# xandercai/JSPSR

Hardware: AMD Instinct MI355X
Metric: Mpixels/sec fwd+bwd, JSPSR x8 on 512^2 DEM tiles (higher is better)
Workload: dtype bf16; 1 GPU; jspsr_r8_img_msk (image+mask guided, 43.87M params), 8 x 512x512 tiles per GPU, train step (fwd + L1/L2/Sobel loss + bwd + grad all-reduce + AdamW); storage policy: bf16 activations / gradients / MFMA operands, fp32 accumulation, BatchNorm statistics, master weights and optimizer, and the generator head (affinity logits + offsets) kept as fp32 planes; tiles_per_gpu=8, tile=512, global_tiles=8, parallelism=dp1, step_mode=eager

## Files before the change

### include/jspsr_hip.h

```cpp
#ifndef JSPSR_HIP_H
#define JSPSR_HIP_H

#include <stddef.h>
#include <stdint.h>

#ifdef __cplusplus
extern "C" {
#endif

#define JSPSR_OK 0
#define JSPSR_EINVAL (-1)
#define JSPSR_EALIGN (-2)

typedef void* jspsr_stream_t;

int jspsr_abi_version(void);
long long jspsr_launch_count(const char* what);
int jspsr_conv_dynamic_queue(int on);
const char* jspsr_last_error(void);

int jspsr_prop_forward_f32(const float* dem, const float* weight, const float* offset,
                           int offset_channels, const float* wk, const float* b0, float scale,
                           float* out, int B, int H, int W, jspsr_stream_t stream);

// ... 105 lines not shown
                       const void* red_x, int red_cstride, const float* red_par, float* red_out, jspsr_stream_t stream);

size_t jspsr_conv2d_wgrad_workspace_bytes(int dtype, int B, int OH, int OW, int Cg, int Cx, int KH, int KW);
int jspsr_conv2d_wgrad_x_affine_ok(int dtype, int B, int OH, int OW, int Cg, int Cx, int KH, int KW, int stride, int pad);
int jspsr_conv2d_wgrad(int dtype, const void* G, int Cg, int g_cstride, int g_coff, const void* X, int Cx,
                       int x_cstride, int x_coff, float* dW, int R, int C, int B, int OH, int OW,
                       int IH, int IW, int KH, int KW, int stride, int pad, int accumulate,
                       const float* x_affine, int x_relu, void* workspace, jspsr_stream_t stream);
int jspsr_conv2d_wgrad_scaled(int dtype, const void* G, int Cg, int g_cstride, int g_coff, const void* X, int Cx,
                              int x_cstride, int x_coff, float* dW, int R, int C, int B, int OH, int OW,
                              int IH, int IW, int KH, int KW, int stride, int pad, int accumulate,
                              const float* x_scale, int x_scale_bstride, void* workspace, jspsr_stream_t stream);

size_t jspsr_reduce_workspace_bytes(int dtype, int C, int nseg);

size_t jspsr_bn_mask_bytes(int dtype, long long npix, int C);
int jspsr_bn_forward(int dtype, const void* x, int x_cs, int x_coff, const void* res, int r_cs, int r_coff,
                     void* y, int y_cs, int y_coff, const float* gamma, const float* beta,
                     float* running_mean, float* running_var, float momentum, float eps, int training,
                     int relu, float res_scale, float* save_mean, float* save_invstd, long long npix, int C,
                     const float* ext_partial, int ext_rows, const float* res_affine, float* affine_out,
                     void* mask_out, void* workspace, jspsr_stream_t stream);

int jspsr_bn_fold(const float* gamma, const float* beta, const float* running_mean, const float* running_var,
                  float eps, float res_scale, int C, float* scale, float* shift, jspsr_stream_t stream);

int jspsr_bn_reduce_params(const float* gamma, const float* beta, const float* save_mean, const float* save_invstd, int C,
                           float* par, jspsr_stream_t stream);
int jspsr_bn_backward(int dtype, const void* dy, int dy_cs, int dy_coff, const void* y, int y_cs, int y_coff,
                      const void* x, int x_cs, int x_coff, const float* gamma, const float* beta, const float* save_mean,
                      const float* save_invstd, int training, int relu, float res_scale, void* dx, void* dres,
                      float* dgamma, float* dbeta, int accumulate, long long npix, int C, void* workspace,
                      const float* ext_partial, int ext_rows, const void* mask, jspsr_stream_t stream);

int jspsr_act_backward(int dtype, const void* dy, int dy_cs, int dy_coff, const void* y, int y_cs, int relu, void* dz,
                       int dz_cs, float* dbias, long long npix, int C, void* workspace, jspsr_stream_t stream);

int jspsr_gate_pool(int dtype, const void* x, int B, long long npix, int C, float* avg, float* mx, int* amax,
                    void* workspace, jspsr_stream_t stream);
int jspsr_gate_scale(int dtype, const void* x, const float* s, void* y, int B, long long npix, int C,
                     jspsr_stream_t stream);
int jspsr_gate_backward_reduce(int dtype, const void* dy, const void* x, float* ds, int B, long long npix, int C,
                               void* workspace, jspsr_stream_t stream);
int jspsr_gate_backward_apply(int dtype, const void* dy, const float* s, const float* davg, const float* dmax,
                              const int* amax, void* dx, int B, long long npix, int C, jspsr_stream_t stream);

size_t jspsr_loss_workspace_bytes(int B, int H, int W);
int jspsr_loss_forward(const float* pred, const float* gt, float w1, float w2, float wg, float* losses,
                       void* workspace, int B, int H, int W, jspsr_stream_t stream);
int jspsr_loss_backward(const float* pred, const float* gt, const float* grad_total, float w1, float w2,
                        float wg, float* grad_pred, const void* workspace, int B, int H, int W,
                        jspsr_stream_t stream);

size_t jspsr_loss_menu_workspace_bytes(int terms, int planes, int H, int W);
int jspsr_loss_menu_forward(const float* pred, const float* gt, int terms, int planes, int H, int W, int n_keys,
                            const int* key_slot, const double* key_weight, const float* base_losses, float* out,
                            void* workspace, jspsr_stream_t stream);
int jspsr_loss_menu_backward(const float* pred, const float* gt, int terms, int planes, int H, int W,
                             const double* slot_weight, const float* grad_total, float* grad_pred,
                             const void* workspace, jspsr_stream_t stream);
size_t jspsr_loss_valid_workspace_bytes(int B, int H, int W);
int jspsr_loss_valid_forward(const float* pred, const float* gt, const unsigned char* valid, float w1, float w2, float wg,
                             float* losses, void* workspace, int B, int H, int W, jspsr_stream_t stream);
int jspsr_loss_valid_backward(const float* pred, const float* gt, const unsigned char* valid, const float* grad_total,
                              float w1, float w2, float wg, float* grad_pred, const void* workspace, int B, int H, int W,
                              jspsr_stream_t stream);
// ... 124 lines not shown
```

### jspsr_amd/_lib.py

```python
from __future__ import annotations

import ctypes
import os
import subprocess
import threading

_HERE = os.path.dirname(os.path.abspath(__file__))
SO_PATH = os.environ.get("JSPSR_LAB_LIB") or os.path.join(_HERE, "lib", "libjspsr_hip.so")
CSRC = os.path.join(_HERE, "csrc")
ABI_VERSION = 25

_lock = threading.Lock()
_lib = None

c_p = ctypes.c_void_p
c_i = ctypes.c_int
c_f = ctypes.c_float
c_ll = ctypes.c_longlong

SIGNATURES = {
    "jspsr_abi_version": (c_i, []),
    "jspsr_launch_count": (c_ll, [ctypes.c_char_p]),
    "jspsr_conv_dynamic_queue": (c_i, [c_i]),
    "jspsr_last_error": (ctypes.c_char_p, []),
# ... 7 lines not shown
    "jspsr_prop_head_forward": (c_i, [c_i, c_p, c_p, c_p, c_p, c_f, c_p, c_i, c_i, c_i, c_p]),
    "jspsr_prop_head_backward_workspace_bytes": (ctypes.c_size_t, [c_i, c_i, c_i]),
    "jspsr_prop_head_backward": (c_i, [c_i] + [c_p] * 8 + [c_i, c_i, c_i, c_p]),
    "jspsr_prop_logits_forward_f32": (c_i, [c_p, c_p, c_p, c_p, c_f, c_p, c_i, c_i, c_i, c_p]),
    "jspsr_prop_logits_backward_f32": (c_i, [c_p] * 8 + [c_i, c_i, c_i, c_p]),
    "jspsr_head_ok": (c_i, [c_i] * 5),
    "jspsr_head_forward": (c_i, [c_i, c_p, c_i, c_i, c_i, c_p, c_p, c_p, c_i, c_i, c_i, c_p]),
    "jspsr_head_backward_workspace_bytes": (ctypes.c_size_t, [c_i, c_i, c_i]),
    "jspsr_head_backward": (c_i, [c_i, c_p, c_p, c_i, c_p, c_i, c_i, c_p, c_p, c_p, c_i, c_i, c_i, c_p]),
    "jspsr_conv_head1_forward": (c_i, [c_i, c_p, c_i, c_i, c_i, c_p, c_p, c_p, c_i, c_i, c_i, c_p]),
    "jspsr_conv_head1_workspace_bytes": (ctypes.c_size_t, [c_i, c_i, c_i, c_i]),
    "jspsr_conv_head1_backward": (c_i, [c_i, c_p, c_p, c_i, c_i, c_i, c_p, c_p, c_i, c_i, c_p, c_p, c_p, c_i, c_i, c_i, c_p]),
    "jspsr_pack_weight": (c_i, [c_i, c_p, c_p] + [c_i] * 6 + [c_p]),
    "jspsr_pack_chunk": (c_i, []),
    "jspsr_pack_weights_multi": (c_i, [c_p, c_i, c_ll, c_p]),
    "jspsr_conv2d_stats_rows": (c_i, [c_i, c_i, c_i]),
    "jspsr_conv2d_in_affine_ok": (c_i, [c_i] * 5),
    "jspsr_conv2d_forward": (c_i, [c_i] + [c_p] * 4 + [c_i] * 14 + [c_p, c_p, c_p, c_i, c_p, c_i, c_p]),
    "jspsr_conv2d_forward_scaled": (c_i, [c_i] + [c_p] * 4 + [c_i] * 14 + [c_p, c_p, c_p, c_i, c_p, c_i, c_p]),
    "jspsr_bn_fold": (c_i, [c_p, c_p, c_p, c_p, c_f, c_f, c_i, c_p, c_p, c_p]),
    "jspsr_conv2d_dgrad_reduce_ok": (c_i, [c_i] * 10),
    "jspsr_conv2d_dgrad": (c_i, [c_i] + [c_p] * 4 + [c_i] * 16 + [c_p, c_i, c_p, c_p, c_i, c_p, c_p, c_p]),
    "jspsr_conv2d_wgrad_workspace_bytes": (ctypes.c_size_t, [c_i] * 8),
    "jspsr_conv2d_wgrad_x_affine_ok": (c_i, [c_i] * 10),
    "jspsr_conv2d_wgrad": (c_i, [c_i, c_p, c_i, c_i, c_i, c_p, c_i, c_i, c_i, c_p] + [c_i] * 12 + [c_p, c_i, c_p, c_p]),
    "jspsr_conv2d_wgrad_scaled": (c_i, [c_i, c_p, c_i, c_i, c_i, c_p, c_i, c_i, c_i, c_p] + [c_i] * 12 + [c_p, c_i, c_p, c_p]),
    "jspsr_reduce_workspace_bytes": (ctypes.c_size_t, [c_i, c_i, c_i]),
    "jspsr_bn_forward": (c_i, [c_i, c_p, c_i, c_i, c_p, c_i, c_i, c_p, c_i, c_i, c_p, c_p, c_p, c_p, c_f, c_f, c_i,
                               c_i, c_f, c_p, c_p, c_ll, c_i, c_p, c_i, c_p, c_p, c_p, c_p, c_p]),
    "jspsr_bn_mask_bytes": (ctypes.c_size_t, [c_i, c_ll, c_i]),
    "jspsr_bn_reduce_params": (c_i, [c_p, c_p, c_p, c_p, c_i, c_p, c_p]),
    "jspsr_bn_backward": (c_i, [c_i, c_p, c_i, c_i, c_p, c_i, c_i, c_p, c_i, c_i, c_p, c_p, c_p, c_p, c_i, c_i, c_f,
                                c_p, c_p, c_p, c_p, c_i, c_ll, c_i, c_p, c_p, c_i, c_p, c_p]),
    "jspsr_act_backward": (c_i, [c_i, c_p, c_i, c_i, c_p, c_i, c_i, c_p, c_i, c_p, c_ll, c_i, c_p, c_p]),
    "jspsr_gate_pool": (c_i, [c_i, c_p, c_i, c_ll, c_i, c_p, c_p, c_p, c_p, c_p]),
    "jspsr_gate_scale": (c_i, [c_i, c_p, c_p, c_p, c_i, c_ll, c_i, c_p]),
    "jspsr_gate_backward_reduce": (c_i, [c_i, c_p, c_p, c_p, c_i, c_ll, c_i, c_p, c_p]),
    "jspsr_gate_backward_apply": (c_i, [c_i, c_p, c_p, c_p, c_p, c_p, c_p, c_i, c_ll, c_i, c_p]),
    "jspsr_loss_workspace_bytes": (ctypes.c_size_t, [c_i, c_i, c_i]),
    "jspsr_loss_forward": (c_i, [c_p, c_p, c_f, c_f, c_f, c_p, c_p, c_i, c_i, c_i, c_p]),
    "jspsr_loss_backward": (c_i, [c_p, c_p, c_p, c_f, c_f, c_f, c_p, c_p, c_i, c_i, c_i, c_p]),
    "jspsr_loss_menu_workspace_bytes": (ctypes.c_size_t, [c_i, c_i, c_i, c_i]),
    "jspsr_loss_menu_forward": (c_i, [c_p, c_p, c_i, c_i, c_i, c_i, c_i, c_p, c_p, c_p, c_p, c_p, c_p]),
    "jspsr_loss_menu_backward": (c_i, [c_p, c_p, c_i, c_i, c_i, c_i, c_p, c_p, c_p, c_p, c_p]),
    "jspsr_loss_valid_workspace_bytes": (ctypes.c_size_t, [c_i, c_i, c_i]),
    "jspsr_loss_valid_forward": (c_i, [c_p, c_p, c_p, c_f, c_f, c_f, c_p, c_p, c_i, c_i, c_i, c_p]),
    "jspsr_loss_valid_backward": (c_i, [c_p, c_p, c_p, c_p, c_f, c_f, c_f, c_p, c_p, c_i, c_i, c_i, c_p]),
    "jspsr_loss_menu_valid_workspace_bytes": (ctypes.c_size_t, [c_i, c_i, c_i, c_i]),
    "jspsr_loss_menu_valid_forward": (c_i, [c_p, c_p, c_p, c_i, c_i, c_i, c_i, c_i, c_p, c_p, c_p, c_p, c_p, c_p]),
    "jspsr_loss_menu_valid_backward": (c_i, [c_p, c_p, c_p, c_i, c_i, c_i, c_i, c_p, c_p, c_p, c_p, c_p]),
    "jspsr_ssim_workspace_bytes": (ctypes.c_size_t, [c_i, c_i, c_i, c_i]),
    "jspsr_ssim_forward": (c_i, [c_p, c_p, c_i, c_i, c_i, c_i, c_p, c_p, c_p, c_p]),
    "jspsr_metrics_workspace_bytes": (ctypes.c_size_t, [c_i, c_i]),
    "jspsr_metrics_forward": (c_i, [c_p, c_p, c_i, c_i, c_f, c_f, c_f, c_i, c_p, c_p, c_p]),
    "jspsr_scores_batch_workspace_bytes": (ctypes.c_size_t, [c_i, c_i, c_i]),
    "jspsr_scores_batch_forward": (c_i, [c_p, c_p, c_i, c_i, c_i, c_f, c_f, c_f, c_i, c_p, c_p, c_p]),
    "jspsr_scores_batch_valid_workspace_bytes": (ctypes.c_size_t, [c_i, c_i, c_i]),
    "jspsr_scores_batch_valid_forward": (c_i, [c_p, c_p, c_p, c_i, c_i, c_i, c_f, c_f, c_f, c_i, c_p, c_p, c_p, c_p]),
    "jspsr_scenes_assemble_f32": (c_i, [c_p] * 5 + [c_ll] + [c_i] * 6 + [ctypes.c_double, ctypes.c_double, c_p]),
    "jspsr_summary_workspace_bytes": (ctypes.c_size_t, [c_i, c_i, c_ll, c_ll]),
    "jspsr_summary_forward": (c_i, [c_p, c_p, c_i, c_p, c_ll, c_p, c_i, c_p, c_i, c_ll, c_ll, ctypes.c_double, c_p, c_p, c_p]),
    "jspsr_summary_valid_workspace_bytes": (ctypes.c_size_t, [c_i, c_i, c_ll, c_ll]),
    "jspsr_summary_valid_forward": (c_i, [c_p, c_p, c_i, c_p, c_ll, c_p, c_ll, c_p, c_i, c_p, c_i, c_ll, c_ll, ctypes.c_double,
                                          c_p, c_p, c_p, c_p]),
    "jspsr_summary_ranks": (c_i, [c_ll, c_p]),
    "jspsr_errdist_bins": (c_i, [ctypes.c_double, ctypes.c_double, c_p, c_p]),
# ... 86 lines not shown
```

### jspsr_amd/csrc/elementwise.hip

```cpp
#include "common.h"

#include <atomic>
#include <cstdlib>

namespace {

using namespace jspsr;

constexpr int TX = 64, TY = 4;

template <typename T> struct V;
template <> struct V<float> { static constexpr int N = 4; };
template <> struct V<__bf16> { static constexpr int N = 8; };

template <typename T, int N>
struct Pack { T v[N]; };

template <typename T>
__device__ __forceinline__ uint4 load_raw(const T* p) { return *reinterpret_cast<const uint4*>(p); }
template <typename T>
__device__ __forceinline__ void unpack(const uint4& raw, float (&f)[V<T>::N]) {
  if constexpr (sizeof(T) == 4) {
    f[0] = __uint_as_float(raw.x); f[1] = __uint_as_float(raw.y); f[2] = __uint_as_float(raw.z); f[3] = __uint_as_float(raw.w);
  } else {
// ... 109 lines not shown
    long long p = p0 + ty * g.pl + lm.sub;
    for (; p + (PIX_FLY - 1) * step < p1; p += PIX_FLY * step) {
      uint4 raw[PIX_FLY][NTEN];
#pragma unroll
      for (int u = 0; u < PIX_FLY; ++u) load(base + p + u * step, c, raw[u]);
#pragma unroll
      for (int u = 0; u < PIX_FLY; ++u) use(base + p + u * step, c, raw[u], acc);
    }
    for (; p < p1; p += step) {
      uint4 raw[NTEN];
      load(base + p, c, raw);
      use(base + p, c, raw, acc);
    }
  }
#pragma unroll
  for (int k = 0; k < K; ++k)
#pragma unroll
    for (int i = 0; i < N; ++i) red[ty][k][tx * N + i] = acc[k][i];
  __syncthreads();
  if (ty == 0 && lm.sub == 0 && c < g.C) {
    float* dst = partial + ((size_t)blockIdx.x * K) * g.C + c;
#pragma unroll
    for (int k = 0; k < K; ++k)
#pragma unroll
      for (int i = 0; i < N; ++i) {
        float s = 0.f;
        for (int j = 0; j < g.pl; ++j)
#pragma unroll
          for (int y = 0; y < TY; ++y) s += red[y][k][(tx + j * g.lpp) * N + i];
        dst[(size_t)k * g.C + i] = s;
      }
  }
}
template <typename T, int NTEN, typename L, typename F>
__device__ __forceinline__ void for_pixels_mlp(const RedGeom& g, L&& load, F&& use) {
  constexpr int N = V<T>::N;
  const LaneMap lm = lane_map<N>(g);
  const int c = lm.c;
  if (c >= g.C) return;
  const int seg = blockIdx.x / g.chunks, chunk = blockIdx.x % g.chunks;
  const long long p0 = chunk * g.chunk_pix;
  const long long p1 = (p0 + g.chunk_pix < g.npix) ? p0 + g.chunk_pix : g.npix;
  const long long step = TY * g.pl, base = (long long)seg * g.npix;
  long long p = p0 + threadIdx.y * g.pl + lm.sub;
  for (; p + (PIX_FLY - 1) * step < p1; p += PIX_FLY * step) {
    uint4 raw[PIX_FLY][NTEN];
#pragma unroll
    for (int u = 0; u < PIX_FLY; ++u) load(base + p + u * step, c, raw[u]);
#pragma unroll
    for (int u = 0; u < PIX_FLY; ++u) use(p + u * step, base + p + u * step, c, raw[u]);
  }
  for (; p < p1; p += step) {
    uint4 raw[NTEN];
    load(base + p, c, raw);
    use(p, base + p, c, raw);
  }
}

template <int N>
__device__ __forceinline__ void load_param(const float* __restrict__ p, float (&f)[N]) {
#pragma unroll
  for (int i = 0; i < N; i += 4) {
    const float4 v = *reinterpret_cast<const float4*>(p + i);
    f[i] = v.x; f[i + 1] = v.y; f[i + 2] = v.z; f[i + 3] = v.w;
  }
}

__device__ __forceinline__ double wave_sum_rows(const float* __restrict__ partial, int rows, size_t pitch, size_t off) {
  const int lane = threadIdx.x & 63;
  double s = 0.0;
  for (int r = lane; r < rows; r += 64) s += (double)partial[(size_t)r * pitch + off];
#pragma unroll
  for (int d = 32; d > 0; d >>= 1) s += __shfl_xor(s, d, 64);
  return s;
}

__device__ __forceinline__ void wave_sum_rows2(const float* __restrict__ partial, int rows, size_t pitch, size_t off0, size_t off1,
                                               double& s0, double& s1) {
  const int lane = threadIdx.x & 63;
  double a = 0.0, b = 0.0;
  int r = lane;
  for (; r + 192 < rows; r += 256) {
    const float x0 = partial[(size_t)r * pitch + off0], x1 = partial[(size_t)(r + 64) * pitch + off0];
// ... 218 lines not shown
  constexpr int N = V<T>::N, NTEN = (RELU == 1 || RELU == 3) ? 3 : 2;
  const int C = g.C, groups = C / N;
  float mu[N], is[N], k0[N], ka[N], kb[N], ga[N], be[N];
  const int c0 = lane_map<N>(g).c;
  if (c0 < C) {
    load_param<N>(mean + c0, mu); load_param<N>(invstd + c0, is);
    load_param<N>(coef + c0, k0); load_param<N>(coef + C + c0, ka); load_param<N>(coef + 2 * C + c0, kb);
    if (RELU == 2) { load_param<N>(gamma + c0, ga); load_param<N>(beta + c0, be); }
  }
  for_pixels_mlp<T, NTEN>(
      g,
      [&](long long pix, int c, uint4 (&raw)[NTEN]) {
        raw[0] = load_raw<T>(dy + (size_t)pix * dy_cs + dy_coff + c);
        raw[1] = load_raw<T>(x + (size_t)pix * x_cs + x_coff + c);
        if constexpr (RELU == 1) raw[2] = load_raw<T>(y + (size_t)pix * y_cs + y_coff + c);
        if constexpr (RELU == 3) raw[2].x = mask[(size_t)pix * groups + c / N];
      },
      [&](long long, long long pix, int c, const uint4 (&raw)[NTEN]) {
        float d[N], xv[N], yv[N], o[N];
        unpack<T>(raw[0], d);
        unpack<T>(raw[1], xv);
        if constexpr (RELU == 1) unpack<T>(raw[2], yv);
#pragma unroll
        for (int k = 0; k < N; ++k) {
          const float xhat = (xv[k] - mu[k]) * is[k];
          const bool off = RELU == 1 ? !(yv[k] > 0.f)
                                     : (RELU == 2 ? !(ga[k] * xhat + be[k] > 0.f) : (RELU == 3 ? !((raw[2].x >> k) & 1u) : false));
          const float dz = off ? 0.f : d[k];
          d[k] = dz;
          o[k] = k0[k] * (dz - ka[k] - xhat * kb[k]);
        }
        store_vec<T>(dx + (size_t)pix * C + c, o);
        if (dres) store_vec<T>(dres + (size_t)pix * C + c, d);
      });
}

template <typename T, bool RELU>
__global__ __launch_bounds__(TX * TY) void act_bwd_kernel(const T* __restrict__ dy, int dy_cs, int dy_coff,
                                                         const T* __restrict__ y, int y_cs, int relu,
                                                         T* __restrict__ dz, int dz_cs, RedGeom g,
                                                         float* __restrict__ partial) {
  constexpr int N = V<T>::N;
  constexpr int NTEN = RELU ? 2 : 1;
  (void)relu;
  reduce_pixels_mlp<T, 1, NTEN>(
      g, partial,
      [&](long long pix, int c, uint4 (&raw)[NTEN]) {
        raw[0] = load_raw<T>(dy + (size_t)pix * dy_cs + dy_coff + c);
        if constexpr (RELU) raw[1] = load_raw<T>(y + (size_t)pix * y_cs + c);
      },
      [&](long long pix, int c, const uint4 (&raw)[NTEN], float (&acc)[1][N]) {
        float d[N], yv[N];
        unpack<T>(raw[0], d);
        if constexpr (RELU) unpack<T>(raw[1], yv);
#pragma unroll
        for (int i = 0; i < N; ++i) {
          if (RELU && !(yv[i] > 0.f)) d[i] = 0.f;
          acc[0][i] += d[i];
        }
        if (dz) store_vec<T>(dz + (size_t)pix * dz_cs + c, d);
      });
}

__global__ void sum_rows_kernel(const float* __restrict__ partial, int rows, int K, int k, int C, float* __restrict__ out) {
  const int c = blockIdx.x * (blockDim.x >> 6) + (threadIdx.x >> 6);
  if (c >= C) return;
// ... 307 lines not shown
    if (ext_rows <= 0) return fail(JSPSR_EINVAL, "bn_backward: ext_rows must be positive");
    if (ext_rows > 1024) {
      rows = g.chunks < 1024 ? (g.chunks > 0 ? g.chunks : 1) : 1024;
      hipLaunchKernelGGL(fold_rows_kernel, dim3(rows, (2 * C + 255) / 256), dim3(256), 0, s, ext_partial, ext_rows, 2 * C, rows, partial);
      if (int e = check_launch("bn_fold_rows")) return e;
    } else {
      partial = const_cast<float*>(ext_partial);
      rows = ext_rows;
    }
  } else {
    if (mode == 0) { BN_BWD_REDUCE(0, false); }
    else if (mode == 2) { BN_BWD_REDUCE(2, false); }
    else if (mode == 1) { if (premask) { BN_BWD_REDUCE(1, true); } else { BN_BWD_REDUCE(1, false); } }
    else { if (premask) { BN_BWD_REDUCE(3, true); } else { BN_BWD_REDUCE(3, false); } }
    if (int e = check_launch("bn_bwd_reduce")) return e;
  }
#undef BN_BWD_REDUCE
  hipLaunchKernelGGL(bn_bwd_finalize_kernel, dim3((C + 3) / 4), dim3(256), 0, s, partial, rows, C, npix, gamma,
                     save_invstd, training, res_scale, accumulate, dgamma, dbeta, coef);
  if (int e = check_launch("bn_bwd_finalize")) return e;
#define BN_BWD_APPLY(R, DY, CS, OFF, DRES) DISPATCH(dtype, hipLaunchKernelGGL((bn_bwd_apply_kernel<T, R>), red_grid(g, vec), dim3(TX, TY), 0, s, \
                                     static_cast<const T*>(DY), CS, OFF, static_cast<const T*>(y), y_cs, y_coff,            \
                                     static_cast<const T*>(x), x_cs, x_coff, save_mean, save_invstd, gamma, beta, coef, mk, \
                                     static_cast<T*>(dx), static_cast<T*>(DRES), g))
  if (premask) { BN_BWD_APPLY(0, dres, C, 0, nullptr); }
  else if (mode == 0) { BN_BWD_APPLY(0, dy, dy_cs, dy_coff, dres); }
  else if (mode == 1) { BN_BWD_APPLY(1, dy, dy_cs, dy_coff, dres); }
  else if (mode == 2) { BN_BWD_APPLY(2, dy, dy_cs, dy_coff, dres); }
  else { BN_BWD_APPLY(3, dy, dy_cs, dy_coff, dres); }
#undef BN_BWD_APPLY
  return check_launch("bn_bwd_apply");
}

extern "C" int jspsr_bn_fold(const float* gamma, const float* beta, const float* running_mean, const float* running_var,
                             float eps, float res_scale, int C, float* scale, float* shift, jspsr_stream_t stream) {
  if (!gamma || !beta || !running_mean || !running_var || !scale || !shift || C <= 0)
    return fail(JSPSR_EINVAL, "bn_fold: bad arguments");
  hipLaunchKernelGGL(bn_fold_kernel, dim3((C + 255) / 256), dim3(256), 0, static_cast<hipStream_t>(stream), gamma, beta,
                     running_mean, running_var, eps, res_scale, C, scale, shift);
  return check_launch("bn_fold");
}

extern "C" int jspsr_act_backward(int dtype, const void* dy, int dy_cs, int dy_coff, const void* y, int y_cs, int relu,
                                  void* dz, int dz_cs, float* dbias, long long npix, int C, void* workspace,
                                  jspsr_stream_t stream) {
  if (int e = check_c(dtype, C, "act_backward")) return e;
  if (!dy || (relu && !y) || !workspace || npix <= 0) return fail(JSPSR_EINVAL, "act_backward: null pointer or empty tensor");
  const int vec = dtype == JSPSR_F32 ? 4 : 8;
  if (dy_cs % vec || dy_coff % vec || (dz && dz_cs % vec) || (relu && (y_cs % vec || y_cs < C)))
    return fail(JSPSR_EINVAL, "act_backward: bad pitch");
  hipStream_t s = static_cast<hipStream_t>(stream);
  float* partial = static_cast<float*>(workspace);
  const RedGeom g = make_red(npix, 1, C, vec);
#define ACT_BWD(R) DISPATCH(dtype, hipLaunchKernelGGL((act_bwd_kernel<T, R>), red_grid(g, vec), dim3(TX, TY), 0, s, static_cast<const T*>(dy), \
                                     dy_cs, dy_coff, static_cast<const T*>(y), y_cs, relu, static_cast<T*>(dz), dz_cs, g, partial))
  if (relu) { ACT_BWD(true); } else { ACT_BWD(false); }
#undef ACT_BWD
  if (int e = check_launch("act_backward")) return e;
  if (dbias) {
    hipLaunchKernelGGL(sum_rows_kernel, dim3((C + 3) / 4), dim3(256), 0, s, partial, g.chunks, 1, 0, C, dbias);
    return check_launch("act_backward_bias");
  }
  return JSPSR_OK;
}

extern "C" int jspsr_gate_pool(int dtype, const void* x, int B, long long npix, int C, float* avg, float* mx, int* amax,
// ... 395 lines not shown
```

### jspsr_amd/kernels.py

```python
from __future__ import annotations

import torch

from . import _lib

F32, BF16 = 0, 1


def _dt(t: torch.Tensor) -> int:
    if t.dtype == torch.float32:
        return F32
    if t.dtype == torch.bfloat16:
        return BF16
    raise TypeError(f"unsupported dtype {t.dtype}")


def epc(dtype: torch.dtype) -> int:
    return 4 if dtype == torch.float32 else 8


def _stream() -> int:
    return torch.cuda.current_stream().cuda_stream


# ... 153 lines not shown
                 x_affine=None, x_relu=False, x_scale=None):
    _chk_s(G, "conv2d_wgrad")
    _chk_s(X, "conv2d_wgrad")
    B, OH, OW, Cg_ = G.shape
    _, IH, IW, Cx_ = X.shape
    Cgs, Cxs = pitch(G), pitch(X)
    cg = Cg_ if cg is None else cg
    cx = Cx_ if cx is None else cx
    if out is None:
        out = torch.empty((R, C, KH, KW), dtype=torch.float32, device=G.device)
    lib = _lib.load()
    dt = _dt(G)
    nbytes = lib.jspsr_conv2d_wgrad_workspace_bytes(dt, B, OH, OW, cg, cx, KH, KW)
    ws = torch.empty(max(nbytes, 16), dtype=torch.uint8, device=G.device)
    head = (dt, G.data_ptr(), cg, Cgs, g_coff, X.data_ptr(), cx, Cxs, x_coff, out.data_ptr(), R, C, B, OH, OW, IH, IW, KH, KW,
            stride, pad, int(accumulate))
    if x_scale is not None:
        if x_affine is not None:
            raise ValueError("conv2d_wgrad: x_scale and x_affine exclude each other")
        _chk_scale(x_scale, B, cx, "conv2d_wgrad x_scale")
        _lib.check(lib.jspsr_conv2d_wgrad_scaled(*head, x_scale.data_ptr(), x_scale.shape[1], ws.data_ptr(), _stream()),
                   "jspsr_conv2d_wgrad_scaled")
    else:
        _lib.check(lib.jspsr_conv2d_wgrad(*head, x_affine.data_ptr() if x_affine is not None else None, int(x_relu),
                                          ws.data_ptr(), _stream()), "jspsr_conv2d_wgrad")
    return out



_ws_cache = {}


def _workspace(dtype_code: int, C: int, nseg: int, device) -> torch.Tensor:
    lib = _lib.load()
    n = lib.jspsr_reduce_workspace_bytes(dtype_code, C, nseg)
    key = (device, _stream())
    buf = _ws_cache.get(key)
    if buf is None or buf.numel() < n:
        buf = torch.empty(max(n, 1 << 20), dtype=torch.uint8, device=device)
        _ws_cache[key] = buf
    return buf


def bn_forward(x, gamma, beta, running_mean, running_var, momentum, eps, training, relu=False, res=None,
               res_scale=1.0, out=None, out_coff=0, partial=None, res_affine=None, stats_only=False, want_mask=False):
    _chk_s(x, "bn_forward")
    B, H, W, C = x.shape
    affine = torch.empty((2, C), dtype=torch.float32, device=x.device) if stats_only else None
    if out is None and not stats_only:
        out = torch.empty((B, H, W, C), dtype=x.dtype, device=x.device)
    mean = torch.empty(C, dtype=torch.float32, device=x.device)
    invstd = torch.empty(C, dtype=torch.float32, device=x.device)
    dt = _dt(x)
    ws = _workspace(dt, C, 1, x.device)
    lib = _lib.load()
    mask = torch.empty(lib.jspsr_bn_mask_bytes(dt, B * H * W, C), dtype=torch.uint8, device=x.device) if want_mask else None
    _lib.check(lib.jspsr_bn_forward(dt, x.data_ptr(), pitch(x), 0, res.data_ptr() if res is not None else None,
                                    pitch(res) if res is not None else 0, 0, out.data_ptr() if out is not None else None,
                                    pitch(out) if out is not None else 0, out_coff,
                                    gamma.data_ptr(), beta.data_ptr(),
                                    running_mean.data_ptr() if running_mean is not None else None,
                                    running_var.data_ptr() if running_var is not None else None,
                                    float(momentum), float(eps), int(training), int(relu), float(res_scale),
                                    mean.data_ptr(), invstd.data_ptr(), B * H * W, C,
                                    partial.data_ptr() if partial is not None else None,
                                    partial.shape[0] if partial is not None else 0,
                                    res_affine.data_ptr() if res_affine is not None else None,
                                    affine.data_ptr() if affine is not None else None,
# ... 18 lines not shown
                grads_into=None, ext_partial=None, mask=None):
    _chk_s(dy, "bn_backward")
    B, H, W, C = x.shape
    dx = torch.empty((B, H, W, C), dtype=x.dtype, device=x.device)
    dres = torch.empty((B, H, W, C), dtype=x.dtype, device=x.device) if want_dres else None
    if grads_into is not None:
        dgamma, dbeta = grads_into
        for t in (dgamma, dbeta):
            if t.dtype != torch.float32 or not t.is_contiguous() or t.numel() != C or not t.is_cuda:
                raise ValueError("bn_backward: grads_into buffers must be contiguous fp32 of C elements on the GPU")
    else:
        dgamma = torch.empty(C, dtype=torch.float32, device=x.device)
        dbeta = torch.empty(C, dtype=torch.float32, device=x.device)
    dt = _dt(x)
    ws = _workspace(dt, C, 1, x.device)
    lib = _lib.load()
    if mask is not None and (mask.dtype != torch.uint8 or not mask.is_contiguous() or
                             mask.numel() != lib.jspsr_bn_mask_bytes(dt, B * H * W, C)):
        raise ValueError("bn_backward: mask is not the bit mask bn_forward(want_mask=True) made for this shape")
    _lib.check(lib.jspsr_bn_backward(dt, dy.data_ptr(), pitch(dy), 0, y.data_ptr() if y is not None else None,
                                     pitch(y) if y is not None else 0, 0, x.data_ptr(), pitch(x), 0, gamma.data_ptr(),
                                     beta.data_ptr() if beta is not None else None,
                                     mean.data_ptr(), invstd.data_ptr(), int(training), int(relu), float(res_scale),
                                     dx.data_ptr(), dres.data_ptr() if dres is not None else None, dgamma.data_ptr(),
                                     dbeta.data_ptr(), int(grads_into is not None), B * H * W, C, ws.data_ptr(),
                                     ext_partial.data_ptr() if ext_partial is not None else None,
                                     ext_partial.shape[0] if ext_partial is not None else 0,
                                     mask.data_ptr() if mask is not None else None, _stream()), "jspsr_bn_backward")
    if grads_into is not None:
        return dx, dres, None, None
    return dx, dres, dgamma, dbeta


def act_backward(dy, y, relu, want_dz=True, want_dbias=True, dz_channels=None):
    _chk_s(dy, "act_backward")
    B, H, W, C = dy.shape
    dz = None
    if want_dz:
        cz = C if dz_channels is None else dz_channels
        dz = torch.empty((B, H, W, cz), dtype=dy.dtype, device=dy.device) if cz == C else \
            torch.zeros((B, H, W, cz), dtype=dy.dtype, device=dy.device)
    dbias = torch.empty(C, dtype=torch.float32, device=dy.device) if want_dbias else None
    dt = _dt(dy)
    ws = _workspace(dt, C, 1, dy.device)
    lib = _lib.load()
    if y is not None:
        y = nhwc(y)
    _lib.check(lib.jspsr_act_backward(dt, dy.data_ptr(), pitch(dy), 0, y.data_ptr() if y is not None else None,
                                      pitch(y) if y is not None else 0, int(relu),
                                      dz.data_ptr() if dz is not None else None, dz.shape[3] if dz is not None else 0,
                                      dbias.data_ptr() if dbias is not None else None, B * H * W, C, ws.data_ptr(),
                                      _stream()), "jspsr_act_backward")
    return dz, dbias


def gate_pool(x):
    _chk(x, "gate_pool")
    B, H, W, C = x.shape
    avg = torch.empty((B, C), dtype=torch.float32, device=x.device)
    mx = torch.empty_like(avg)
    amax = torch.empty((B, C), dtype=torch.int32, device=x.device)
    dt = _dt(x)
    ws = _workspace(dt, C, B, x.device)
    lib = _lib.load()
    _lib.check(lib.jspsr_gate_pool(dt, x.data_ptr(), B, H * W, C, avg.data_ptr(), mx.data_ptr(), amax.data_ptr(),
                                   ws.data_ptr(), _stream()), "jspsr_gate_pool")
# ... 71 lines not shown
```

### jspsr_amd/ops.py

```python
from __future__ import annotations

import collections
import os
import weakref

import torch

from . import _lib
from . import kernels as K


def _stream() -> int:
    return torch.cuda.current_stream().cuda_stream


def _need_gpu(*ts):
    for t in ts:
        if not t.is_cuda:
            raise RuntimeError("jspsr_amd ops run on the GPU only (got a CPU tensor); there is no CPU fallback")
        if t.dtype != torch.float32:
            raise TypeError(f"expected float32, got {t.dtype}")


def prop_forward_raw(dem, weight, offset, w, b, scale, out):
# ... 465 lines not shown
    _, table, grand = _pack_table
    _lib.check(_lib.load().jspsr_pack_weights_multi(table.data_ptr(), len(entries), grand, _stream()), "jspsr_pack_weights_multi")
    for p, mode, c_pad, dtype, packed in entries:
        p.__dict__["_jspsr_packs"][(mode, c_pad, dtype, p.data_ptr())] = (packed, (p._version, _weights_epoch))
    return len(entries)


def pad_channels(x: torch.Tensor, mult: int) -> torch.Tensor:
    c = x.shape[-1]
    p = (-c) % mult
    return x if p == 0 else torch.nn.functional.pad(x, (0, p))


def _wgrad_into(param, G, X, R, C, KH, KW, stride, pad, **kw):
    gbuf = param.grad if param is not None and getattr(param, "_jspsr_direct_grad", False) else None
    if (gbuf is not None and gbuf.dtype == torch.float32 and gbuf.is_contiguous() and gbuf.is_cuda
            and tuple(gbuf.shape) == (R, C, KH, KW)):
        K.conv2d_wgrad(G, X, R, C, KH, KW, stride, pad, out=gbuf, accumulate=True, **kw)
        ready = getattr(param, "_jspsr_grad_ready", None)
        if ready is not None:
            ready(param)
        return None
    return K.conv2d_wgrad(G, X, R, C, KH, KW, stride, pad, **kw)


_aux_streams = {}
_marks = {}
RUN_AHEAD = int(os.environ.get("JSPSR_RUN_AHEAD", "16"))
wgrad_async = os.environ.get("JSPSR_WGRAD_ASYNC", "1") != "0"
wgrad_after_dgrad = os.environ.get("JSPSR_WGRAD_AFTER_DGRAD", "0") != "0"
wgrad_one_stream = os.environ.get("JSPSR_WGRAD_ONE_STREAM", "0") != "0"
bn_reduce_fused = os.environ.get("JSPSR_BN_REDUCE_FUSE", "1") != "0"
bn_relu_mask = os.environ.get("JSPSR_BN_RELU_MASK", "1") != "0"


def aux_streams():
    return list(_aux_streams.values())


def _wgrad_async(param, G, X, R, C, KH, KW, stride, pad, **kw):
    if not wgrad_async:
        return _wgrad_into(param, G, X, R, C, KH, KW, stride, pad, **kw)
    cur = torch.cuda.current_stream()
    key = 0 if wgrad_one_stream else cur.cuda_stream
    aux = _aux_streams.get(key)
    if aux is None:
        aux = _aux_streams[key] = torch.cuda.Stream(device=G.device)
    aux.wait_stream(cur)
    with torch.cuda.stream(aux):
        dW = _wgrad_into(param, G, X, R, C, KH, KW, stride, pad, **kw)
    for t_ in kw.values():
        if isinstance(t_, torch.Tensor):
            t_.record_stream(aux)
    G.record_stream(aux)
    X.record_stream(aux)
    if not torch.cuda.is_current_stream_capturing():
        marks = _marks.setdefault(cur.cuda_stream, collections.deque())
        marks.append(cur.record_event())
        if len(marks) > RUN_AHEAD:
            marks.popleft().synchronize()
    if dW is not None:
        cur.wait_stream(aux)
        dW.record_stream(cur)
    return dW


# ... 249 lines not shown
                r = zd
            else:
                zd, r, md, idd = conv_bn(x, wdd, 1, stride, 0, gdd, bdd, rmd, rvd, momd, epsd, trd, False, par=wd)
                r_aff = None
        else:
            r_aff = None
            if stride != 1 or O != I:
                raise ValueError("res_unit: identity shortcut needs stride 1 and equal channel counts")
            wdd = gdd = bdd = zd = md = idd = None
            trd = False
            r = x
        out_v = dest[0].slice(dest[1], O, z1.shape[:3]) if dest is not None else None
        masked = bool(act) and bn_relu_mask
        z2, out, m2, i2, *mk2 = conv_bn(z1 if fuse1 else y1, w2d, 3, 1, 1, g2d, b2d, rm2, rv2, mom2, eps2, tr2, bool(act), r, float(scale),
                                        out_v, par=w2, res_affine=r_aff, in_affine=aff1, want_mask=masked)
        ctx.cfg = (stride, float(scale), bool(act), has_d, tr1, tr2, trd)
        ctx.wparams = tuple(p if isinstance(p, torch.nn.Parameter) else None for p in (w1, w2, wd))
        ctx.bparams = tuple(p if isinstance(p, torch.nn.Parameter) else None for p in (g1, b1, g2, b2, gd, bd))
        ctx.save_for_backward(x, w1d, g1d, b1d, z1, m1, i1, y1, w2d, g2d, b2d, z2, m2, i2, out if act and not masked else None,
                              wdd, gdd, bdd, zd, md, idd, aff1, mk2[0] if masked else None)
        return out

    @staticmethod
    def backward(ctx, dout):
        stride, scale, act, has_d, tr1, tr2, trd = ctx.cfg
        (x, w1, g1, b1, z1, m1, i1, y1, w2, g2, b2, z2, m2, i2, out, wd, gd, bd, zd, md, idd, aff1, mask2) = ctx.saved_tensors
        cdt = x.dtype
        B, H, W, Cin = x.shape
        O = w1.shape[0]
        dout = K.nhwc(dout)
        need_x = ctx.needs_input_grad[0]
        pg1, pb1, pg2, pb2, pgd, pbd = ctx.bparams
        sink2, sink1 = _bn_sink(pg2, pb2), _bn_sink(pg1, pb1)
        dz2, dres, dg2, db2 = K.bn_backward(dout, out, z2, g2, m2, i2, tr2, 1 if act else 0, scale,
                                            want_dres=(need_x or has_d), beta=b2, grads_into=sink2, mask=mask2)
        if sink2 is not None:
            _bn_ready(pg2, pb2)
        if dres is None:
            dres = dout
        p1, p2, pd = ctx.wparams

        def wgrad2():
            if aff1 is not None:
                return _wgrad_async(p2, dz2, z1, O, O, 3, 3, 1, 1, x_affine=aff1, x_relu=True)
            return _wgrad_async(p2, dz2, y1, O, O, 3, 3, 1, 1)

        if not wgrad_after_dgrad:
            dW2 = wgrad2()
        Bz, Hz, Wz, _ = z1.shape
        part1 = None
        if bn_reduce_fused and tr1 and K.dgrad_reduce_ok(cdt, Bz, Hz, Wz, O, O, 3, 3, 1, 1) and z1.is_contiguous():
            par1 = K.bn_reduce_params(g1, b1, m1, i1)
            dy1, part1 = K.conv2d_dgrad(dz2, _packed(p2, w2, 1, O, cdt), z1.shape[1:3], 1, 1, red=(z1, par1))
        else:
            dy1 = K.conv2d_dgrad(dz2, _packed(p2, w2, 1, O, cdt), z1.shape[1:3], 1, 1)
        if wgrad_after_dgrad:
            dW2 = wgrad2()
        del dz2
        dz1, _, dg1, db1 = K.bn_backward(dy1, None, z1, g1, m1, i1, tr1, 2, 1.0, beta=b1, grads_into=sink1, ext_partial=part1)
        if sink1 is not None:
            _bn_ready(pg1, pb1)
        del dy1
        dW1 = None if wgrad_after_dgrad else _wgrad_async(p1, dz1, x, O, Cin, 3, 3, stride, 1)
        dWd = dgd = dbd = None
        side = dres
        deposit = None
        if isinstance(ctx.grad_extra, tuple):
            holder, off, n = ctx.grad_extra
            if holder.deferred is not None and has_d and need_x:
                cur = torch.cuda.current_stream()
                cur.wait_event(holder.deferred_event)
                deposit = holder.deferred.narrow(3, off, n)
                if tuple(deposit.shape) != tuple(x.shape):
                    raise RuntimeError(f"res_unit: parked gradient slice {tuple(deposit.shape)} does not match the input {tuple(x.shape)}")
                if deposit.dtype != x.dtype or not (deposit.is_contiguous() or K.is_slice(deposit)):
                    holder.pending_deposits -= 1
                    deposit = None
                else:
                    deposit.record_stream(cur)
            elif holder.deferred is not None:
                holder.pending_deposits -= 1
        extra = ctx.grad_extra.take_deferred() if (ctx.grad_extra is not None and not isinstance(ctx.grad_extra, tuple)) else deposit
        if extra is not None:
            extra = K.nhwc(extra)
            if tuple(extra.shape) != tuple(x.shape):
                raise RuntimeError(f"res_unit: deferred gradient {tuple(extra.shape)} does not match the input {tuple(x.shape)}")
            if not (has_d and need_x):
                side, extra = side + extra, None
        if has_d:
            sinkd = _bn_sink(pgd, pbd)
            dzd, _, dgd, dbd = K.bn_backward(dres, None, zd, gd, md, idd, trd, 0, 1.0, beta=bd, grads_into=sinkd)
            if sinkd is not None:
                _bn_ready(pgd, pbd)
            dWd = _wgrad_async(pd, dzd, x, O, Cin, 1, 1, stride, 0)
            side = K.conv2d_dgrad(dzd, _packed(pd, wd, 1, O, cdt), (H, W), stride, 0, addend=extra) if need_x else None
        dx = None
        if need_x and deposit is not None:
            K.conv2d_dgrad(dz1, _packed(p1, w1, 1, O, cdt), (H, W), stride, 1, addend=K.nhwc(side), out=deposit)
            ctx.grad_extra[0].deposit_events.append(torch.cuda.current_stream().record_event())
        elif need_x:
            dx = K.conv2d_dgrad(dz1, _packed(p1, w1, 1, O, cdt), (H, W), stride, 1, addend=K.nhwc(side))
        if wgrad_after_dgrad:
            dW1 = _wgrad_async(p1, dz1, x, O, Cin, 3, 3, stride, 1)
        return (dx, dW1, dg1, db1, dW2, dg2, db2, dWd, dgd, dbd, None, None, None, None, None, None)


def conv_bn_infer(x, weight, gamma, beta, bn, stride, pad, relu=False, res=None, res_scale=1.0, dest=None):
    x = K.nhwc(x)
    rm, rv, _, eps, training = bn
    if training or rm is None:
        raise RuntimeError("conv_bn_infer: BatchNorm must be in eval mode with running statistics")
    sc, sh = K.bn_fold(gamma.detach(), beta.detach(), rm, rv, eps, res_scale if res is not None else 1.0)
    O, I, KH, KW = weight.shape
    B, H, W, Cp = x.shape
    out = None
    if dest is not None:
        out = dest[0].slice(dest[1], O, (B, (H + 2 * pad - KH) // stride + 1, (W + 2 * pad - KW) // stride + 1))
    return K.conv2d_forward(x, _packed(weight, weight.detach().contiguous(), 0, Cp, x.dtype), sh, stride, pad, relu, out=out,
                            scale=sc, addend=K.nhwc(res) if res is not None else None)


def conv_transpose_bn_infer(x, weight, gamma, beta, bn, relu=True, dest=None):
    x = K.nhwc(x)
    rm, rv, _, eps, training = bn
# ... 127 lines not shown
```

Before: 36.64 Mpixel/s.

## Fuse residual-unit output BN and shortcut BN backward into one paired kernel set

In residual units with a downsample shortcut, the backward passes of the second BN and the shortcut BN now run through a single reduce/finalize/apply sequence. That sequence reads dy, the ReLU mask and both pre-BN inputs once. This avoids materialising dres and running a second full BN backward pass over the same gradient. It adds a wider kernel that carries more live registers per thread and more per-channel parameters. It also changes how dgd/dbd and the side gradient are threaded through the Python backward.

```diff
diff --git a/include/jspsr_hip.h b/include/jspsr_hip.h
--- a/include/jspsr_hip.h
+++ b/include/jspsr_hip.h
@@ -161,6 +161,14 @@
                       const float* save_invstd, int training, int relu, float res_scale, void* dx, void* dres,
                       float* dgamma, float* dbeta, int accumulate, long long npix, int C, void* workspace,
                       const float* ext_partial, int ext_rows, const void* mask, jspsr_stream_t stream);
+
+size_t jspsr_bn_backward_pair_workspace_bytes(int dtype, int C);
+int jspsr_bn_backward_pair(int dtype, const void* dy, int dy_cs, int dy_coff, const void* mask, const void* x2, int x2_cs,
+                           int x2_coff, const float* gamma2, const float* save_mean2, const float* save_invstd2,
+                           int training2, float res_scale, const void* xd, int xd_cs, int xd_coff, const float* gammad,
+                           const float* save_meand, const float* save_invstdd, int trainingd, void* dx2, void* dxd,
+                           float* dgamma2, float* dbeta2, int accumulate2, float* dgammad, float* dbetad, int accumulated,
+                           long long npix, int C, void* workspace, jspsr_stream_t stream);
 
 int jspsr_act_backward(int dtype, const void* dy, int dy_cs, int dy_coff, const void* y, int y_cs, int relu, void* dz,
                        int dz_cs, float* dbias, long long npix, int C, void* workspace, jspsr_stream_t stream);
diff --git a/jspsr_amd/_lib.py b/jspsr_amd/_lib.py
--- a/jspsr_amd/_lib.py
+++ b/jspsr_amd/_lib.py
@@ -63,6 +63,9 @@
     "jspsr_bn_reduce_params": (c_i, [c_p, c_p, c_p, c_p, c_i, c_p, c_p]),
     "jspsr_bn_backward": (c_i, [c_i, c_p, c_i, c_i, c_p, c_i, c_i, c_p, c_i, c_i, c_p, c_p, c_p, c_p, c_i, c_i, c_f,
                                 c_p, c_p, c_p, c_p, c_i, c_ll, c_i, c_p, c_p, c_i, c_p, c_p]),
+    "jspsr_bn_backward_pair_workspace_bytes": (ctypes.c_size_t, [c_i, c_i]),
+    "jspsr_bn_backward_pair": (c_i, [c_i, c_p, c_i, c_i, c_p, c_p, c_i, c_i, c_p, c_p, c_p, c_i, c_f, c_p, c_i, c_i, c_p, c_p, c_p, c_i,
+                                     c_p, c_p, c_p, c_p, c_i, c_p, c_p, c_i, c_ll, c_i, c_p, c_p]),
     "jspsr_act_backward": (c_i, [c_i, c_p, c_i, c_i, c_p, c_i, c_i, c_p, c_i, c_p, c_ll, c_i, c_p, c_p]),
     "jspsr_gate_pool": (c_i, [c_i, c_p, c_i, c_ll, c_i, c_p, c_p, c_p, c_p, c_p]),
     "jspsr_gate_scale": (c_i, [c_i, c_p, c_p, c_p, c_i, c_ll, c_i, c_p]),
diff --git a/jspsr_amd/csrc/elementwise.hip b/jspsr_amd/csrc/elementwise.hip
--- a/jspsr_amd/csrc/elementwise.hip
+++ b/jspsr_amd/csrc/elementwise.hip
@@ -165,7 +165,7 @@
       }
   }
 }
-template <typename T, int NTEN, typename L, typename F>
+template <typename T, int NTEN, int FLY = PIX_FLY, typename L, typename F>
 __device__ __forceinline__ void for_pixels_mlp(const RedGeom& g, L&& load, F&& use) {
   constexpr int N = V<T>::N;
   const LaneMap lm = lane_map<N>(g);
@@ -176,12 +176,12 @@
   const long long p1 = (p0 + g.chunk_pix < g.npix) ? p0 + g.chunk_pix : g.npix;
   const long long step = TY * g.pl, base = (long long)seg * g.npix;
   long long p = p0 + threadIdx.y * g.pl + lm.sub;
-  for (; p + (PIX_FLY - 1) * step < p1; p += PIX_FLY * step) {
-    uint4 raw[PIX_FLY][NTEN];
-#pragma unroll
-    for (int u = 0; u < PIX_FLY; ++u) load(base + p + u * step, c, raw[u]);
-#pragma unroll
-    for (int u = 0; u < PIX_FLY; ++u) use(p + u * step, base + p + u * step, c, raw[u]);
+  for (; p + (FLY - 1) * step < p1; p += FLY * step) {
+    uint4 raw[FLY][NTEN];
+#pragma unroll
+    for (int u = 0; u < FLY; ++u) load(base + p + u * step, c, raw[u]);
+#pragma unroll
+    for (int u = 0; u < FLY; ++u) use(p + u * step, base + p + u * step, c, raw[u]);
   }
   for (; p < p1; p += step) {
     uint4 raw[NTEN];
@@ -466,6 +466,123 @@
         }
         store_vec<T>(dx + (size_t)pix * C + c, o);
         if (dres) store_vec<T>(dres + (size_t)pix * C + c, d);
+      });
+}
+
+template <typename T>
+__global__ __launch_bounds__(TX * TY) void bn_bwd_reduce_pair_kernel(const T* __restrict__ dy, int dy_cs, int dy_coff,
+                                                                    const unsigned char* __restrict__ mask,
+                                                                    const T* __restrict__ x2, int x2_cs, int x2_coff,
+                                                                    const float* __restrict__ mean2, const float* __restrict__ invstd2,
+                                                                    const T* __restrict__ xd, int xd_cs, int xd_coff,
+                                                                    const float* __restrict__ meand, const float* __restrict__ invstdd,
+                                                                    RedGeom g, float* __restrict__ partial) {
+  constexpr int N = V<T>::N;
+  const int groups = g.C / N;
+  float mu2[N], is2[N], mud[N], isd[N];
+  const int c0 = lane_map<N>(g).c;
+  if (c0 < g.C) {
+    load_param<N>(mean2 + c0, mu2); load_param<N>(invstd2 + c0, is2);
+    load_param<N>(meand + c0, mud); load_param<N>(invstdd + c0, isd);
+  }
+  reduce_pixels_mlp<T, 3, 4>(
+      g, partial,
+      [&](long long pix, int c, uint4 (&raw)[4]) {
+        raw[0] = load_raw<T>(dy + (size_t)pix * dy_cs + dy_coff + c);
+        raw[1] = load_raw<T>(x2 + (size_t)pix * x2_cs + x2_coff + c);
+        raw[2] = load_raw<T>(xd + (size_t)pix * xd_cs + xd_coff + c);
+        raw[3].x = mask[(size_t)pix * groups + c / N];
+      },
+      [&](long long, int, const uint4 (&raw)[4], float (&acc)[3][N]) {
+        float d[N], xv[N], xw[N];
+        const unsigned m = raw[3].x;
+        unpack<T>(raw[0], d);
+        unpack<T>(raw[1], xv);
+        unpack<T>(raw[2], xw);
+#pragma unroll
+        for (int i = 0; i < N; ++i) {
+          const float xhat = (xv[i] - mu2[i]) * is2[i];
+          const float xhatd = (xw[i] - mud[i]) * isd[i];
+          const float dz = !((m >> i) & 1u) ? 0.f : d[i];
+          acc[0][i] += dz;
+          acc[1][i] += dz * xhat;
+          acc[2][i] += dz * xhatd;
+        }
+      });
+}
+
+__global__ void bn_bwd_finalize_pair_kernel(const float* __restrict__ partial, int rows, int C, long long count,
+                                            const float* __restrict__ gamma2, const float* __restrict__ invstd2, int training2,
+                                            float res_scale, int accumulate2, float* __restrict__ dgamma2, float* __restrict__ dbeta2,
+                                            const float* __restrict__ gammad, const float* __restrict__ invstdd, int trainingd,
+                                            int accumulated, float* __restrict__ dgammad, float* __restrict__ dbetad,
+                                            float* __restrict__ coef) {
+  const int c = blockIdx.x * (blockDim.x >> 6) + (threadIdx.x >> 6);
+  if (c >= C) return;
+  double s, sx;
+  wave_sum_rows2(partial, rows, (size_t)3 * C, c, (size_t)C + c, s, sx);
+  const double sd = wave_sum_rows(partial, rows, (size_t)3 * C, (size_t)2 * C + c);
+  if ((threadIdx.x & 63) != 0) return;
+  auto layer = [&](double sxl, const float* gamma, const float* invstd, int training, float rs, int accumulate,
+                   float* dgamma, float* dbeta, float* co) {
+    dbeta[c] = (accumulate ? dbeta[c] : 0.f) + (float)(s * rs);
+    dgamma[c] = (accumulate ? dgamma[c] : 0.f) + (float)(sxl * rs);
+    const float k = gamma[c] * invstd[c] * rs;
+    co[c] = k;
+    co[C + c] = training ? (float)(s / (double)count) : 0.f;
+    co[2 * C + c] = training ? (float)(sxl / (double)count) : 0.f;
+  };
+  layer(sx, gamma2, invstd2, training2, res_scale, accumulate2, dgamma2, dbeta2, coef);
+  layer(sd, gammad, invstdd, trainingd, 1.0f, accumulated, dgammad, dbetad, coef + 3 * C);
+}
+
+#ifndef K4_PAIR_APPLY_FLY
+#define K4_PAIR_APPLY_FLY 1
+#endif
+constexpr int PAIR_APPLY_FLY = K4_PAIR_APPLY_FLY;
+template <typename T>
+__global__ __launch_bounds__(TX * TY) void bn_bwd_apply_pair_kernel(const T* __restrict__ dy, int dy_cs, int dy_coff,
+                                                                   const unsigned char* __restrict__ mask,
+                                                                   const T* __restrict__ x2, int x2_cs, int x2_coff,
+                                                                   const float* __restrict__ mean2, const float* __restrict__ invstd2,
+                                                                   const T* __restrict__ xd, int xd_cs, int xd_coff,
+                                                                   const float* __restrict__ meand, const float* __restrict__ invstdd,
+                                                                   const float* __restrict__ coef, T* __restrict__ dx2,
+                                                                   T* __restrict__ dxd, RedGeom g) {
+  constexpr int N = V<T>::N;
+  const int C = g.C, groups = C / N;
+  float mu2[N], is2[N], k2[N], a2[N], b2[N], mud[N], isd[N], kd[N], ad[N], bd[N];
+  const int c0 = lane_map<N>(g).c;
+  if (c0 < C) {
+    load_param<N>(mean2 + c0, mu2); load_param<N>(invstd2 + c0, is2);
+    load_param<N>(coef + c0, k2); load_param<N>(coef + C + c0, a2); load_param<N>(coef + 2 * C + c0, b2);
+    load_param<N>(meand + c0, mud); load_param<N>(invstdd + c0, isd);
+    load_param<N>(coef + 3 * C + c0, kd); load_param<N>(coef + 4 * C + c0, ad); load_param<N>(coef + 5 * C + c0, bd);
+  }
+  for_pixels_mlp<T, 4, PAIR_APPLY_FLY>(
+      g,
+      [&](long long pix, int c, uint4 (&raw)[4]) {
+        raw[0] = load_raw<T>(dy + (size_t)pix * dy_cs + dy_coff + c);
+        raw[1] = load_raw<T>(x2 + (size_t)pix * x2_cs + x2_coff + c);
+        raw[2] = load_raw<T>(xd + (size_t)pix * xd_cs + xd_coff + c);
+        raw[3].x = mask[(size_t)pix * groups + c / N];
+      },
+      [&](long long, long long pix, int c, const uint4 (&raw)[4]) {
+        float d[N], xv[N], xw[N], o[N], od[N];
+        const unsigned m = raw[3].x;
+        unpack<T>(raw[0], d);
+        unpack<T>(raw[1], xv);
+        unpack<T>(raw[2], xw);
+#pragma unroll
+        for (int k = 0; k < N; ++k) {
+          const float xhat = (xv[k] - mu2[k]) * is2[k];
+          const float xhatd = (xw[k] - mud[k]) * isd[k];
+          const float dz = !((m >> k) & 1u) ? 0.f : d[k];
+          o[k] = k2[k] * (dz - a2[k] - xhat * b2[k]);
+          od[k] = kd[k] * (dz - ad[k] - xhatd * bd[k]);
+        }
+        store_vec<T>(dx2 + (size_t)pix * C + c, o);
+        store_vec<T>(dxd + (size_t)pix * C + c, od);
       });
 }
 
@@ -839,6 +956,50 @@
   return check_launch("bn_bwd_apply");
 }
 
+extern "C" size_t jspsr_bn_backward_pair_workspace_bytes(int dtype, int C) {
+  const size_t base = jspsr_reduce_workspace_bytes(dtype, C, 1);
+  return base ? base + (size_t)2 * C * sizeof(float) : 0;
+}
+
+extern "C" int jspsr_bn_backward_pair(int dtype, const void* dy, int dy_cs, int dy_coff, const void* mask, const void* x2, int x2_cs,
+                                      int x2_coff, const float* gamma2, const float* save_mean2, const float* save_invstd2,
+                                      int training2, float res_scale, const void* xd, int xd_cs, int xd_coff, const float* gammad,
+                                      const float* save_meand, const float* save_invstdd, int trainingd, void* dx2, void* dxd,
+                                      float* dgamma2, float* dbeta2, int accumulate2, float* dgammad, float* dbetad, int accumulated,
+                                      long long npix, int C, void* workspace, jspsr_stream_t stream) {
+  if (int e = check_c(dtype, C, "bn_backward_pair")) return e;
+  if (!dy || !mask || !x2 || !gamma2 || !save_mean2 || !save_invstd2 || !xd || !gammad || !save_meand || !save_invstdd || !dx2 ||
+      !dxd || !dgamma2 || !dbeta2 || !dgammad || !dbetad || !workspace || npix <= 0)
+    return fail(JSPSR_EINVAL, "bn_backward_pair: null pointer or empty tensor");
+  const int vec = dtype == JSPSR_F32 ? 4 : 8;
+  if (dy_cs % vec || dy_coff % vec || x2_cs % vec || x2_coff % vec || xd_cs % vec || xd_coff % vec)
+    return fail(JSPSR_EINVAL, "bn_backward_pair: channel pitches/offsets must be multiples of %d", vec);
+  if (dy_coff < 0 || x2_coff < 0 || xd_coff < 0 || dy_cs < dy_coff + C || x2_cs < x2_coff + C || xd_cs < xd_coff + C)
+    return fail(JSPSR_EINVAL, "bn_backward_pair: a channel slice of %d channels does not fit its pitch", C);
+  if (dx2 == dxd || dgamma2 == dgammad || dbeta2 == dbetad)
+    return fail(JSPSR_EINVAL, "bn_backward_pair: the two layers' outputs must be distinct");
+  for (const void* p : {dy, x2, xd, (const void*)dx2, (const void*)dxd, (const void*)workspace})
+    if (reinterpret_cast<uintptr_t>(p) % 16) return fail(JSPSR_EALIGN, "bn_backward_pair: tensors and workspace must be 16-byte aligned");
+  hipStream_t s = static_cast<hipStream_t>(stream);
+  float* coef = static_cast<float*>(workspace);
+  float* partial = coef + 6 * C;
+  const RedGeom g = make_red(npix, 1, C, vec);
+  const unsigned char* mk = static_cast<const unsigned char*>(mask);
+  DISPATCH(dtype, hipLaunchKernelGGL(bn_bwd_reduce_pair_kernel<T>, red_grid(g, vec), dim3(TX, TY), 0, s, static_cast<const T*>(dy), dy_cs,
+                                     dy_coff, mk, static_cast<const T*>(x2), x2_cs, x2_coff, save_mean2, save_invstd2,
+                                     static_cast<const T*>(xd), xd_cs, xd_coff, save_meand, save_invstdd, g, partial));
+  if (int e = check_launch("bn_bwd_reduce_pair")) return e;
+  hipLaunchKernelGGL(bn_bwd_finalize_pair_kernel, dim3((C + 3) / 4), dim3(256), 0, s, partial, g.chunks, C, npix, gamma2, save_invstd2,
+                     training2, res_scale, accumulate2, dgamma2, dbeta2, gammad, save_invstdd, trainingd, accumulated, dgammad, dbetad,
+                     coef);
+  if (int e = check_launch("bn_bwd_finalize_pair")) return e;
+  DISPATCH(dtype, hipLaunchKernelGGL(bn_bwd_apply_pair_kernel<T>, red_grid(g, vec), dim3(TX, TY), 0, s, static_cast<const T*>(dy), dy_cs,
+                                     dy_coff, mk, static_cast<const T*>(x2), x2_cs, x2_coff, save_mean2, save_invstd2,
+                                     static_cast<const T*>(xd), xd_cs, xd_coff, save_meand, save_invstdd, coef, static_cast<T*>(dx2),
+                                     static_cast<T*>(dxd), g));
+  return check_launch("bn_bwd_apply_pair");
+}
+
 extern "C" int jspsr_bn_fold(const float* gamma, const float* beta, const float* running_mean, const float* running_var,
                              float eps, float res_scale, int C, float* scale, float* shift, jspsr_stream_t stream) {
   if (!gamma || !beta || !running_mean || !running_var || !scale || !shift || C <= 0)
diff --git a/jspsr_amd/kernels.py b/jspsr_amd/kernels.py
--- a/jspsr_amd/kernels.py
+++ b/jspsr_amd/kernels.py
@@ -209,8 +209,10 @@
 
 
 def _workspace(dtype_code: int, C: int, nseg: int, device) -> torch.Tensor:
-    lib = _lib.load()
-    n = lib.jspsr_reduce_workspace_bytes(dtype_code, C, nseg)
+    return _workspace_bytes(_lib.load().jspsr_reduce_workspace_bytes(dtype_code, C, nseg), device)
+
+
+def _workspace_bytes(n: int, device) -> torch.Tensor:
     key = (device, _stream())
     buf = _ws_cache.get(key)
     if buf is None or buf.numel() < n:
@@ -295,6 +297,43 @@
     return dx, dres, dgamma, dbeta
 
 
+def bn_backward_pair(dy, mask, x2, gamma2, mean2, invstd2, training2, res_scale, xd, gammad, meand, invstdd, trainingd,
+                     grads_into2=None, grads_intod=None):
+    _chk_s(dy, "bn_backward_pair")
+    _chk_s(x2, "bn_backward_pair")
+    _chk_s(xd, "bn_backward_pair")
+    B, H, W, C = x2.shape
+    if tuple(xd.shape) != (B, H, W, C) or tuple(dy.shape) != (B, H, W, C) or xd.dtype != x2.dtype or dy.dtype != x2.dtype:
+        raise ValueError(f"bn_backward_pair: dy {tuple(dy.shape)} {dy.dtype}, x2 {tuple(x2.shape)} {x2.dtype} and xd "
+                         f"{tuple(xd.shape)} {xd.dtype} must agree")
+    dx2 = torch.empty((B, H, W, C), dtype=x2.dtype, device=x2.device)
+    dxd = torch.empty((B, H, W, C), dtype=x2.dtype, device=x2.device)
+    sinks = []
+    for into in (grads_into2, grads_intod):
+        if into is not None:
+            for t in into:
+                if t.dtype != torch.float32 or not t.is_contiguous() or t.numel() != C or not t.is_cuda:
+                    raise ValueError("bn_backward_pair: grads_into buffers must be contiguous fp32 of C elements on the GPU")
+            sinks.append(tuple(into))
+        else:
+            sinks.append((torch.empty(C, dtype=torch.float32, device=x2.device), torch.empty(C, dtype=torch.float32, device=x2.device)))
+    dt = _dt(x2)
+    lib = _lib.load()
+    if mask is None or mask.dtype != torch.uint8 or not mask.is_contiguous() or mask.numel() != lib.jspsr_bn_mask_bytes(dt, B * H * W, C):
+        raise ValueError("bn_backward_pair: mask is not the bit mask bn_forward(want_mask=True) made for this shape")
+    ws = _workspace_bytes(lib.jspsr_bn_backward_pair_workspace_bytes(dt, C), x2.device)
+    _lib.check(lib.jspsr_bn_backward_pair(dt, dy.data_ptr(), pitch(dy), 0, mask.data_ptr(), x2.data_ptr(), pitch(x2), 0,
+                                          gamma2.data_ptr(), mean2.data_ptr(), invstd2.data_ptr(), int(training2), float(res_scale),
+                                          xd.data_ptr(), pitch(xd), 0, gammad.data_ptr(), meand.data_ptr(), invstdd.data_ptr(),
+                                          int(trainingd), dx2.data_ptr(), dxd.data_ptr(), sinks[0][0].data_ptr(), sinks[0][1].data_ptr(),
+                                          int(grads_into2 is not None), sinks[1][0].data_ptr(), sinks[1][1].data_ptr(),
+                                          int(grads_intod is not None), B * H * W, C, ws.data_ptr(), _stream()),
+               "jspsr_bn_backward_pair")
+    g2 = (None, None) if grads_into2 is not None else sinks[0]
+    gd = (None, None) if grads_intod is not None else sinks[1]
+    return dx2, dxd, g2[0], g2[1], gd[0], gd[1]
+
+
 def act_backward(dy, y, relu, want_dz=True, want_dbias=True, dz_channels=None):
     _chk_s(dy, "act_backward")
     B, H, W, C = dy.shape
diff --git a/jspsr_amd/ops.py b/jspsr_amd/ops.py
--- a/jspsr_amd/ops.py
+++ b/jspsr_amd/ops.py
@@ -521,6 +521,7 @@
 wgrad_one_stream = os.environ.get("JSPSR_WGRAD_ONE_STREAM", "0") != "0"
 bn_reduce_fused = os.environ.get("JSPSR_BN_REDUCE_FUSE", "1") != "0"
 bn_relu_mask = os.environ.get("JSPSR_BN_RELU_MASK", "1") != "0"
+bn_shortcut_merge = os.environ.get("JSPSR_BN_SHORTCUT_MERGE", "1") != "0"
 
 
 def aux_streams():
@@ -836,11 +837,18 @@
         need_x = ctx.needs_input_grad[0]
         pg1, pb1, pg2, pb2, pgd, pbd = ctx.bparams
         sink2, sink1 = _bn_sink(pg2, pb2), _bn_sink(pg1, pb1)
-        dz2, dres, dg2, db2 = K.bn_backward(dout, out, z2, g2, m2, i2, tr2, 1 if act else 0, scale,
-                                            want_dres=(need_x or has_d), beta=b2, grads_into=sink2, mask=mask2)
+        paired = bn_shortcut_merge and has_d and act and mask2 is not None
+        if paired:
+            sinkd = _bn_sink(pgd, pbd)
+            dz2, dzd, dg2, db2, dgd, dbd = K.bn_backward_pair(dout, mask2, z2, g2, m2, i2, tr2, scale, zd, gd, md, idd, trd,
+                                                              grads_into2=sink2, grads_intod=sinkd)
+            dres = None
+        else:
+            dz2, dres, dg2, db2 = K.bn_backward(dout, out, z2, g2, m2, i2, tr2, 1 if act else 0, scale,
+                                                want_dres=(need_x or has_d), beta=b2, grads_into=sink2, mask=mask2)
         if sink2 is not None:
             _bn_ready(pg2, pb2)
-        if dres is None:
+        if dres is None and not paired:
             dres = dout
         p1, p2, pd = ctx.wparams
 
@@ -866,7 +874,9 @@
             _bn_ready(pg1, pb1)
         del dy1
         dW1 = None if wgrad_after_dgrad else _wgrad_async(p1, dz1, x, O, Cin, 3, 3, stride, 1)
-        dWd = dgd = dbd = None
+        dWd = None
+        if not paired:
+            dgd = dbd = None
         side = dres
         deposit = None
         if isinstance(ctx.grad_extra, tuple):
@@ -890,10 +900,11 @@
             if tuple(extra.shape) != tuple(x.shape):
                 raise RuntimeError(f"res_unit: deferred gradient {tuple(extra.shape)} does not match the input {tuple(x.shape)}")
             if not (has_d and need_x):
-                side, extra = side + extra, None
+                side, extra = (side + extra if side is not None else None), None
         if has_d:
-            sinkd = _bn_sink(pgd, pbd)
-            dzd, _, dgd, dbd = K.bn_backward(dres, None, zd, gd, md, idd, trd, 0, 1.0, beta=bd, grads_into=sinkd)
+            if not paired:
+                sinkd = _bn_sink(pgd, pbd)
+                dzd, _, dgd, dbd = K.bn_backward(dres, None, zd, gd, md, idd, trd, 0, 1.0, beta=bd, grads_into=sinkd)
             if sinkd is not None:
                 _bn_ready(pgd, pbd)
             dWd = _wgrad_async(pd, dzd, x, O, Cin, 1, 1, stride, 0)
```

New measurement: 37.06 Mpixel/s (median of 6 runs). 1.1% higher.
